# dalek-cryptography/zkp

Hardware: AMD Instinct MI355X
Metric: proofs/sec + batch-verifies/sec, CMZ13 10-attr credential, 1/2/4/8 MI355X (higher is better)
Workload: dtype u32x9 (29-bit limbs, u64 accumulate)

## Files before the change

zkp_amd/csrc/comb_tables.h:

```cpp
#pragma once
#include "quad.h"
#include "stmt_pairs.h"

namespace zkp {

template <int TEETH>
struct comb_cfg {
  static_assert(TEETH == 4 || TEETH == 8 || TEETH == 16 || TEETH == 32, "teeth");
  static constexpr int BITS = 256 / TEETH;
  static constexpr int WINDOWS = BITS / 4;
  static constexpr int ENTRIES = 8 * TEETH + 1;
};
constexpr int comb_entries(int teeth) { return 8 * teeth + 1; }
constexpr int LADDER_ENTRIES = 8;

__device__ __forceinline__ void q_store_cached(dev_ext* dst, const qcached& c, int q) {
  uint32_t* w = reinterpret_cast<uint32_t*>(dst) + 9 * q;
#pragma unroll
  for (int i = 0; i < 9; ++i) w[i] = c.c.v[i];
}

__global__ void __launch_bounds__(256)
k_comb_slots(uint32_t n_points, const uint32_t* __restrict__ uses, uint32_t comb_min, uint32_t group_min, uint32_t max_tables,
             uint32_t* __restrict__ counter, uint32_t* __restrict__ slot_of, uint32_t* __restrict__ slot_pt, uint32_t* __restrict__ group_start,
// ... 468 lines not shown
  ge_identity(acc);
  ge_identity(lo);
  issue(0);
  auto pick = [&](uint32_t& c0, uint32_t& c1, ge_cached& sel, uint32_t& neg) {
    const uint32_t nib = c0 & 15u;
    c0 = __builtin_amdgcn_alignbit(c1, c0, 4);
    c1 >>= 4;
    neg = (uint32_t)(nib < 8u);
    const uint32_t mag = neg ? 8u - nib : nib - 8u;
    const uint32_t row = mag ? run * GROUP_ROW_CHUNKS + (mag - 1u) * 9u : (uint32_t)GROUP_IDENT_ROW;
    const uint4* ent = lds + (size_t)row * 16 + col;
    uint32_t wd[36];
#pragma unroll
    for (int q = 0; q < 9; ++q) {
      const uint4 x = ent[q * 16];
      wd[4 * q + 0] = x.x; wd[4 * q + 1] = x.y; wd[4 * q + 2] = x.z; wd[4 * q + 3] = x.w;
    }
    fe_set(sel.YmX, wd); fe_set(sel.YpX, wd + 9); fe_set(sel.Z2, wd + 18); fe_set(sel.T2d, wd + 27);
  };
#pragma unroll 1
  for (int pass = 0; pass < 2; ++pass) {
    if (live && pass) { ge_double4(acc); ge_double4(lo); }
    uint32_t alo = pass ? dlo[2] : dlo[3], ahi = pass ? dhi[2] : dhi[3];
    uint32_t blo = pass ? dlo[0] : dlo[1], bhi = pass ? dhi[0] : dhi[1];
#pragma unroll 1
    for (int j = 0; j < 16; ++j) {
      asm volatile("s_waitcnt vmcnt(0)\n\ts_barrier" ::: "memory");
      ge_cached sel;
      uint32_t neg = 0;
      if (live) {
        pick(alo, ahi, sel, neg);
        ge_cached_cneg(sel, neg);
        ge_add_cached(acc, acc, sel);
        pick(blo, bhi, sel, neg);
      }
      lds_barrier();
      if (pass == 0 || j != 15) issue((uint32_t)((j + 1) & 15));
      if (live) {
        ge_cached_cneg(sel, neg);
        ge_add_cached(lo, lo, sel);
      }
    }
  }
  if (live) {
    ge_double4(acc);
    ge_double4(acc);
    ge_cached c;
    ge_to_cached(c, lo);
    ge_add_cached(acc, acc, c);
  }
  if (live) {
    ge_cached sel, c;
    ge_cached_identity(sel);
    load_comb_entry(c, comb + (size_t)slot * cfg::ENTRIES + 8 * 16);
    ge_cached_cmov(sel, c, top);
    ge_add_cached(acc, acc, sel);
    store_ext(partial + t, acc);
  }
}

constexpr uint32_t XBAR_RUNS = 8;
constexpr uint32_t XBAR_HALF_TERMS = 31, XBAR_WAVE_TERMS = 2 * XBAR_HALF_TERMS, XBAR_BLOCK_TERMS = 4 * XBAR_WAVE_TERMS;
constexpr int XBAR_WAVE_UINT4 = 9 * 64;
constexpr int XBAR_LDS_UINT4 = 4 * XBAR_WAVE_UINT4;
static_assert(2 + (XBAR_WAVE_TERMS - 2) / GROUP_MIN_USES <= XBAR_RUNS, "a wavefront's consecutive grouped terms must span at most XBAR_RUNS points");
static_assert(2 + (XBAR_HALF_TERMS - 2) / GROUP_MIN_USES <= 4 && XBAR_HALF_TERMS <= 32,
              "the terms of one crossbar service group (a half of the wavefront) must span at most 4 points: sources 32 lanes apart never meet");

__device__ __forceinline__ void comb_group_xbar(uint32_t i0, uint32_t n_g, const uint32_t* __restrict__ list_g, const uint8_t* __restrict__ scalars,
                                                const uint32_t* __restrict__ pidx, const uint32_t* __restrict__ slot_of,
                                                const dev_ext* __restrict__ comb, dev_ext* __restrict__ partial, uint4* lds) {
  using cfg = comb_cfg<16>;
  constexpr uint32_t NONE = 0xffffffffu;
  const uint32_t tid = threadIdx.x, lane = tid & 63u;
  const uint32_t wave = (uint32_t)__builtin_amdgcn_readfirstlane((int)(tid >> 6));
  if (i0 + wave * XBAR_WAVE_TERMS >= n_g) return;
  const uint32_t hl = lane & 31u;
  const uint32_t i = i0 + wave * XBAR_WAVE_TERMS + (lane >> 5) * XBAR_HALF_TERMS + hl;
  const bool listed = hl < XBAR_HALF_TERMS && i < n_g;
  uint32_t t = 0, slot = NONE;
  if (listed) { t = list_g[i]; slot = slot_of[pidx[t]]; }
  uint32_t cur = slot;
  const uint32_t left = (uint32_t)__shfl_up((int)cur, 1);
  if (hl == 31u) cur = left;
  const uint32_t before = (uint32_t)__shfl_up((int)cur, 1);
  const bool change = lane == 0u || (listed && slot != before);
  const uint64_t cm = __ballot(change);
  const uint32_t run = (uint32_t)__popcll(cm & ((2ull << lane) - 1ull)) - 1u;
  const bool live = listed && slot != NONE && run < XBAR_RUNS;
  int first = -1;
  {
    uint64_t mm = cm;
#pragma unroll
    for (uint32_t r = 0; r < XBAR_RUNS; ++r) {
      const int f = mm ? (int)__ffsll((long long)mm) - 1 : -1;
      if ((lane >> 3) == r) first = f;
      mm &= mm - 1ull;
    }
  }
  uint32_t hslot = (uint32_t)__shfl((int)slot, first < 0 ? 0 : first);
  if (first < 0) hslot = NONE;
  const bool have = hslot != NONE;
  const uint4* hsrc = reinterpret_cast<const uint4*>(comb + (size_t)(have ? hslot : 0u) * cfg::ENTRIES + (lane & 7u));
  typedef __attribute__((address_space(1))) const void* gptr_t;
  typedef __attribute__((address_space(3))) void* lptr_t;
  uint4* wlds = lds + (size_t)wave * XBAR_WAVE_UINT4;
  const uint4* mine = wlds + lane;
  auto issue = [&](uint32_t row) {
    const uint4* p = hsrc + (size_t)row * (8 * 9);
    if (have) {
#pragma unroll
      for (int q = 0; q < 9; ++q) __builtin_amdgcn_global_load_lds((gptr_t)(p + q), (lptr_t)(wlds + 64 * q), 16, 0, 0);
    }
  };
  uint32_t dlo[cfg::WINDOWS], dhi[cfg::WINDOWS], top = 0;
  {
    uint32_t sc[8], e[8];
#pragma unroll
    for (int q = 0; q < 8; ++q) sc[q] = 0;
    if (live) load_vec<2>(sc, scalars + 32 * (size_t)t);
    sc_add_pattern(e, top, sc, 0x88888888u);
#pragma unroll
    for (int w = 0; w < cfg::WINDOWS; ++w) {
      uint32_t lo = 0, hi = 0;
#pragma unroll
      for (int m = 0; m < 4; ++m) {
        lo |= (((e[m] >> (4 * w)) & 0xfu) | ((e[m] >> (12 + 4 * w)) & 0xf0u)) << (8 * m);
        hi |= (((e[m + 4] >> (4 * w)) & 0xfu) | ((e[m + 4] >> (12 + 4 * w)) & 0xf0u)) << (8 * m);
      }
      dlo[w] = lo; dhi[w] = hi;
    }
  }
  ge_p3 acc, lo;
  ge_identity(acc);
  ge_identity(lo);
  issue(0);
  const uint32_t run8 = (run & (XBAR_RUNS - 1u)) * 8u;
  auto pick = [&](uint32_t& c0, uint32_t& c1, ge_cached& sel, uint32_t& neg) {
    const uint32_t nib = c0 & 15u;
    c0 = __builtin_amdgcn_alignbit(c1, c0, 4);
    c1 >>= 4;
    neg = (uint32_t)(nib < 8u);
    const uint32_t mag = neg ? 8u - nib : nib - 8u;
    const uint32_t nz = (uint32_t)(mag != 0u);
    const int src = (int)((run8 + mag - nz) << 2);
    uint32_t wd[36];
#pragma unroll
    for (int q = 0; q < 9; ++q) {
      const uint4 x = mine[q * 64];
      wd[4 * q + 0] = xbar_fetch(src, x.x); wd[4 * q + 1] = xbar_fetch(src, x.y);
      wd[4 * q + 2] = xbar_fetch(src, x.z); wd[4 * q + 3] = xbar_fetch(src, x.w);
    }
    const uint32_t m = 0u - nz, id = nz ^ 1u;
#pragma unroll
    for (int q = 0; q < 36; ++q) wd[q] &= m;
    wd[0] |= id; wd[9] |= id; wd[18] |= id << 1;
    fe_set(sel.YmX, wd); fe_set(sel.YpX, wd + 9); fe_set(sel.Z2, wd + 18); fe_set(sel.T2d, wd + 27);
  };
#pragma unroll 1
  for (int pass = 0; pass < 2; ++pass) {
    if (pass) { ge_double4(acc); ge_double4(lo); }
    uint32_t alo = pass ? dlo[2] : dlo[3], ahi = pass ? dhi[2] : dhi[3];
    uint32_t blo = pass ? dlo[0] : dlo[1], bhi = pass ? dhi[0] : dhi[1];
#pragma unroll 1
    for (int j = 0; j < 16; ++j) {
      asm volatile("s_waitcnt vmcnt(0)" ::: "memory");
      ge_cached sel;
      uint32_t neg = 0;
      pick(alo, ahi, sel, neg);
      ge_cached_cneg(sel, neg);
      ge_add_cached(acc, acc, sel);
      pick(blo, bhi, sel, neg);
      asm volatile("s_waitcnt lgkmcnt(0)" ::: "memory");
      if (pass == 0 || j != 15) issue((uint32_t)((j + 1) & 15));
      ge_cached_cneg(sel, neg);
      ge_add_cached(lo, lo, sel);
    }
  }
  ge_double4(acc);
  ge_double4(acc);
  {
    ge_cached c;
    ge_to_cached(c, lo);
    ge_add_cached(acc, acc, c);
  }
  if (live) {
    ge_cached sel, c;
    ge_cached_identity(sel);
    load_comb_entry(c, comb + (size_t)slot * cfg::ENTRIES + 8 * 16);
    ge_cached_cmov(sel, c, top);
    ge_add_cached(acc, acc, sel);
    store_ext(partial + t, acc);
  }
}

constexpr uint32_t LADDER_GROUP_UINT4 = 64u * LADDER_ENTRIES * 9u;
__device__ __forceinline__ void ladder_store_entry(uint4* __restrict__ g, int e, const ge_cached& c) {
  uint32_t w[36];
  fe_get(w, c.YmX); fe_get(w + 9, c.YpX); fe_get(w + 18, c.Z2); fe_get(w + 27, c.T2d);
#pragma unroll
  for (int q = 0; q < 9; ++q) g[(9 * e + q) * 64] = make_uint4(w[4 * q], w[4 * q + 1], w[4 * q + 2], w[4 * q + 3]);
}
__device__ __forceinline__ void ladder_load_entry(ge_cached& c, const uint4* __restrict__ g, uint32_t e) {
  uint32_t w[36];
#pragma unroll
  for (int q = 0; q < 9; ++q) {
    const uint4 v = g[(9u * e + (uint32_t)q) * 64u];
    w[4 * q] = v.x; w[4 * q + 1] = v.y; w[4 * q + 2] = v.z; w[4 * q + 3] = v.w;
  }
  fe_set(c.YmX, w); fe_set(c.YpX, w + 9); fe_set(c.Z2, w + 18); fe_set(c.T2d, w + 27);
}
template <bool CT>
__device__ __forceinline__ void ladder_select(ge_cached& sel, const uint4* __restrict__ g, uint32_t mag) {
  ge_cached_identity(sel);
  if (CT) {
#pragma unroll 1
    for (uint32_t h = 0; h < 4; ++h) {
      ge_cached c0, c1;
      ladder_load_entry(c0, g, 2 * h + 0);
      ladder_load_entry(c1, g, 2 * h + 1);
      ge_cached_cmov(sel, c0, (uint32_t)(mag == 2 * h + 1));
      ge_cached_cmov(sel, c1, (uint32_t)(mag == 2 * h + 2));
    }
  } else if (mag) {
    ladder_load_entry(sel, g, mag - 1);
  }
}

template <bool CT>
__device__ __forceinline__ void term_ladder16(uint32_t t, const uint8_t* __restrict__ scalars, const dev_affine* __restrict__ pt,
                                              uint4* __restrict__ tbl , dev_ext* __restrict__ partial, uint32_t* ecol) {
  uint32_t s[8], e[8], top;
  load_vec<2>(s, scalars + 32 * (size_t)t);
  sc_add_pattern(e, top, s, 0x88888888u);
#pragma unroll
  for (int j = 0; j < 8; ++j) ecol[256 * j] = e[j];
  ge_p3 acc;
  {
    ge_p3 P, m2, m3, m4, m;
    ge_cached c1, c;
    load_affine(P, pt);
    ge_to_cached(c1, P);
    ladder_store_entry(tbl, 0, c1);
    ge_double<true>(m2, P);
    ge_to_cached(c, m2); ladder_store_entry(tbl, 1, c);
    ge_add_cached(m3, m2, c1);
    ge_to_cached(c, m3); ladder_store_entry(tbl, 2, c);
    ge_double<true>(m4, m2);
    ge_to_cached(c, m4); ladder_store_entry(tbl, 3, c);
    ge_add_cached(m, m4, c1);
    ge_to_cached(c, m); ladder_store_entry(tbl, 4, c);
    ge_double<true>(m, m3);
    ge_to_cached(c, m); ladder_store_entry(tbl, 5, c);
    ge_add_cached(m, m, c1);
    ge_to_cached(c, m); ladder_store_entry(tbl, 6, c);
    ge_double<true>(m, m4);
    ge_to_cached(c, m); ladder_store_entry(tbl, 7, c);
    ge_cached sel;
    ge_cached_identity(sel);
    ge_cached_cmov(sel, c1, top);
    ge_identity(acc);
    ge_add_cached(acc, acc, sel);
  }
#pragma unroll 1
  for (int j = 7; j >= 0; --j) {
    uint32_t cur = ecol[256 * j];
#pragma unroll 1
    for (int k = 0; k < 8; ++k) {
      ge_double4(acc);
      const uint32_t nib = cur >> 28;
      cur <<= 4;
      const uint32_t neg = (uint32_t)(nib < 8u);
      const uint32_t mag = neg ? 8u - nib : nib - 8u;
      ge_cached sel;
      ladder_select<CT>(sel, tbl, mag);
      ge_cached_cneg(sel, neg);
      ge_add_cached(acc, acc, sel);
    }
  }
  store_ext(partial + t, acc);
}

__global__ void __launch_bounds__(256, 2)
k_rider_tables(const uint32_t* __restrict__ n_slots, uint32_t max_tables, const uint32_t* __restrict__ slot_pt, const dev_affine* __restrict__ pts,
               dev_ext* __restrict__ comb) {
  __shared__ uint32_t stage[4][36][64];
  __shared__ uint32_t live[4][64];
  const uint32_t wave = threadIdx.x >> 6, lane = threadIdx.x & 63u;
  const uint32_t slot = blockIdx.x * blockDim.x + threadIdx.x, ns = min(*n_slots, max_tables);
  const uint32_t pi = slot < ns ? slot_pt[slot] : 0u;
  const bool have = slot < ns && (pi & STMT_ABSORBED);
  live[wave][lane] = have ? 1u : 0u;
  if (!__ballot(have)) return;
  ge_p3 P, m;
  ge_identity(P);
  if (have) load_affine(P, pts + (pi & ~STMT_ABSORBED));
  dev_ext* tbl0 = comb + (size_t)(slot - lane) * comb_cfg<16>::ENTRIES;
  ge_cached c1, c;
  ge_to_cached(c1, P);
  c = c1;
  m = P;
#pragma unroll 1
  for (int k = 0; k < 128; ++k) {
    if (k == 1) ge_double<true>(m, P);
    else if (k > 1) ge_add_cached(m, m, c1);
    if (k) ge_to_cached(c, m);
    store_entries_staged(stage[wave], live[wave], lane, tbl0, comb_cfg<16>::ENTRIES, (uint32_t)k, c);
  }
}

__device__ __forceinline__ void ladder_build8(uint4* __restrict__ tbl, ge_cached& c1, const dev_affine* __restrict__ pt) {
  ge_p3 P, m2, m3, m4, m;
  ge_cached c;
  load_affine(P, pt);
  ge_to_cached(c1, P);
  ladder_store_entry(tbl, 0, c1);
  ge_double<true>(m2, P);
  ge_to_cached(c, m2); ladder_store_entry(tbl, 1, c);
  ge_add_cached(m3, m2, c1);
  ge_to_cached(c, m3); ladder_store_entry(tbl, 2, c);
  ge_double<true>(m4, m2);
  ge_to_cached(c, m4); ladder_store_entry(tbl, 3, c);
  ge_add_cached(m, m4, c1);
  ge_to_cached(c, m); ladder_store_entry(tbl, 4, c);
  ge_double<true>(m, m3);
  ge_to_cached(c, m); ladder_store_entry(tbl, 5, c);
  ge_add_cached(m, m, c1);
  ge_to_cached(c, m); ladder_store_entry(tbl, 6, c);
  ge_double<true>(m, m4);
  ge_to_cached(c, m); ladder_store_entry(tbl, 7, c);
}
__device__ __forceinline__ void term_ladder16_joint(uint32_t t, uint32_t t2, const uint8_t* __restrict__ scalars, const dev_affine* __restrict__ pt,
                                                    const dev_affine* __restrict__ pt2, uint4* __restrict__ tbl, uint4* __restrict__ tbl2,
                                                    const dev_ext* __restrict__ rider, dev_ext* __restrict__ partial, uint32_t* ecol) {
  uint32_t top, top2;
  {
    uint32_t s[8], e[8];
    load_vec<2>(s, scalars + 32 * (size_t)t);
    sc_add_pattern(e, top, s, 0x88888888u);
#pragma unroll
    for (int j = 0; j < 8; ++j) ecol[256 * j] = e[j];
    load_vec<2>(s, scalars + 32 * (size_t)t2);
    sc_add_pattern(e, top2, s, rider ? 0x80808080u : 0x88888888u);
#pragma unroll
    for (int j = 0; j < 8; ++j) ecol[256 * (8 + j)] = e[j];
  }
  ge_p3 acc;
  ge_identity(acc);
  {
    ge_cached c1;
    ladder_build8(tbl, c1, pt);
    if (top) ge_add_cached(acc, acc, c1);
    if (rider) load_comb_entry(c1, rider);
    else ladder_build8(tbl2, c1, pt2);
    if (top2) ge_add_cached(acc, acc, c1);
  }
#pragma unroll 1
  for (int j = 7; j >= 0; --j) {
    uint32_t cur = ecol[256 * j], cur2 = ecol[256 * (8 + j)];
#pragma unroll 1
    for (int k = 0; k < 8; ++k) {
      ge_double4(acc);
      uint32_t nib = cur >> 28;
      cur <<= 4;
      uint32_t neg = (uint32_t)(nib < 8u);
      uint32_t mag = neg ? 8u - nib : nib - 8u;
      ge_cached sel;
      ladder_select<false>(sel, tbl, mag);
      ge_cached_cneg(sel, neg);
      ge_add_cached(acc, acc, sel);
      if (rider) {
        if (k & 1) {
          const uint32_t v = cur2 >> 24;
          cur2 <<= 8;
          neg = (uint32_t)(v < 128u);
          mag = neg ? 128u - v : v - 128u;
          ge_cached_identity(sel);
          if (mag) load_comb_entry(sel, rider + (mag - 1u));
          ge_cached_cneg(sel, neg);
          ge_add_cached(acc, acc, sel);
        }
      } else {
        nib = cur2 >> 28;
        cur2 <<= 4;
        neg = (uint32_t)(nib < 8u);
        mag = neg ? 8u - nib : nib - 8u;
        ladder_select<false>(sel, tbl2, mag);
        ge_cached_cneg(sel, neg);
        ge_add_cached(acc, acc, sel);
      }
    }
  }
  store_ext(partial + t, acc);
  ge_identity(acc);
  store_ext(partial + t2, acc);
}

}
```

zkp_amd/csrc/fe25519.h:

```cpp
#pragma once
#include <stdint.h>

#if defined(__HIPCC__)
#define ZKP_HD __host__ __device__ __forceinline__
#else
#define ZKP_HD inline
#endif

#if defined(ZKP_HOST_FE51) && !defined(__HIPCC__)
#include "host/fe51.h"
#else

#ifdef ZKP_FE_TRACK
#include <cassert>
#include <cstdio>
#include <cstdlib>
#endif

namespace zkp {

constexpr uint32_t FE_M29 = (1u << 29) - 1;
constexpr uint32_t FE_M23 = (1u << 23) - 1;

struct fe {
  uint32_t v[9];
#ifdef ZKP_FE_TRACK
  uint64_t ub[9];
#endif
};

#ifdef ZKP_FE_TRACK
#define FE_TRACK(stmt) do { stmt; } while (0)
inline void fe_track_fail(const char* what) { fprintf(stderr, "fe bound violation: %s\n", what); abort(); }
inline void fe_set_ub_tight(fe& r) {
  for (int i = 0; i < 8; ++i) r.ub[i] = (1ull << 29) + (1ull << 18);
  r.ub[8] = (1ull << 23) + 16;
}
inline void fe_set_ub_exact(fe& r) { for (int i = 0; i < 9; ++i) r.ub[i] = r.v[i]; }
#else
#define FE_TRACK(stmt) do { } while (0)
#endif

ZKP_HD void fe_0(fe& r) {
#pragma unroll
  for (int i = 0; i < 9; ++i) r.v[i] = 0;
  FE_TRACK(fe_set_ub_exact(r));
}
ZKP_HD void fe_1(fe& r) {
  fe_0(r);
  r.v[0] = 1;
  FE_TRACK(fe_set_ub_exact(r));
}
ZKP_HD void fe_copy(fe& r, const fe& a) { r = a; }

ZKP_HD uint32_t fe_bias2p(int i) { return i == 0 ? 0x3fffffdau : (i == 8 ? 0x00fffffeu : 0x3ffffffeu); }
ZKP_HD uint32_t fe_bias4p(int i) { return i == 0 ? 0x7fffffb4u : (i == 8 ? 0x01fffffcu : 0x7ffffffcu); }

ZKP_HD void fe_add(fe& r, const fe& a, const fe& b) {
#pragma unroll
  for (int i = 0; i < 9; ++i) {
    FE_TRACK(if (a.ub[i] + b.ub[i] > 0xffffffffull) fe_track_fail("fe_add overflow"); r.ub[i] = a.ub[i] + b.ub[i]);
    r.v[i] = a.v[i] + b.v[i];
  }
}

ZKP_HD void fe_sub(fe& r, const fe& a, const fe& b) {
#pragma unroll
  for (int i = 0; i < 9; ++i) {
    FE_TRACK(if (b.ub[i] > fe_bias2p(i)) fe_track_fail("fe_sub: subtrahend exceeds 2p bias");
             if (a.ub[i] + fe_bias2p(i) > 0xffffffffull) fe_track_fail("fe_sub overflow");
             r.ub[i] = a.ub[i] + fe_bias2p(i));
    r.v[i] = a.v[i] + (fe_bias2p(i) - b.v[i]);
  }
}

ZKP_HD void fe_sub4(fe& r, const fe& a, const fe& b) {
#pragma unroll
  for (int i = 0; i < 9; ++i) {
    FE_TRACK(if (b.ub[i] > fe_bias4p(i)) fe_track_fail("fe_sub4: subtrahend exceeds 4p bias");
             if (a.ub[i] + fe_bias4p(i) > 0xffffffffull) fe_track_fail("fe_sub4 overflow");
             r.ub[i] = a.ub[i] + fe_bias4p(i));
    r.v[i] = a.v[i] + (fe_bias4p(i) - b.v[i]);
  }
}

ZKP_HD void fe_neg(fe& r, const fe& a) {
#pragma unroll
  for (int i = 0; i < 9; ++i) {
    FE_TRACK(if (a.ub[i] > fe_bias2p(i)) fe_track_fail("fe_neg: operand exceeds 2p bias"); r.ub[i] = fe_bias2p(i));
    r.v[i] = fe_bias2p(i) - a.v[i];
  }
}

ZKP_HD void fe_carry(fe& r, const fe& a) {
  uint32_t c[9];
#pragma unroll
  for (int i = 0; i < 8; ++i) c[i] = a.v[i] >> 29;
  c[8] = a.v[8] >> 23;
  r.v[0] = (a.v[0] & FE_M29) + 19u * c[8];
#pragma unroll
  for (int i = 1; i < 8; ++i) r.v[i] = (a.v[i] & FE_M29) + c[i - 1];
  r.v[8] = (a.v[8] & FE_M23) + c[7];
  FE_TRACK(fe_set_ub_tight(r));
}

ZKP_HD void fe_cmov(fe& r, const fe& b, uint32_t flag) {
  const bool f = flag != 0;
#pragma unroll
  for (int i = 0; i < 9; ++i) {
    FE_TRACK(if (b.ub[i] > r.ub[i]) r.ub[i] = b.ub[i]);
    r.v[i] = f ? b.v[i] : r.v[i];
  }
}
ZKP_HD void fe_cswap(fe& a, fe& b, uint32_t flag) {
  const bool f = flag != 0;
#pragma unroll
  for (int i = 0; i < 9; ++i) {
    FE_TRACK(uint64_t mx = a.ub[i] > b.ub[i] ? a.ub[i] : b.ub[i]; a.ub[i] = mx; b.ub[i] = mx);
    const uint32_t x = a.v[i], y = b.v[i];
    a.v[i] = f ? y : x;
    b.v[i] = f ? x : y;
  }
}

ZKP_HD void fe_reduce_columns(fe& r, uint64_t c[9]) {
#pragma unroll
  for (int k = 0; k < 8; ++k) {
    c[k + 1] += c[k] >> 29;
    r.v[k] = (uint32_t)c[k] & FE_M29;
  }
  r.v[8] = (uint32_t)c[8] & FE_M23;
  const uint64_t t = c[8] >> 23;
  const uint64_t c0 = (uint64_t)r.v[0] + 19ull * (uint32_t)t;
  r.v[0] = (uint32_t)c0 & FE_M29;
  r.v[1] += (uint32_t)(c0 >> 29) + 152u * (uint32_t)(t >> 32);
  FE_TRACK(fe_set_ub_tight(r));
}

#ifdef ZKP_FE_TRACK
inline void fe_track_mul(const fe& a, const fe& b) {
  unsigned __int128 col[17];
  for (int k = 0; k < 17; ++k) col[k] = 0;
  for (int i = 0; i < 9; ++i) if (a.ub[i] >= (1ull << 31) || b.ub[i] >= (1ull << 31)) fe_track_fail("fe_mul: limb >= 2^31");
  for (int i = 0; i < 9; ++i)
    for (int j = 0; j < 9; ++j) col[i + j] += (unsigned __int128)a.ub[i] * b.ub[j];
  const unsigned __int128 lim = ((unsigned __int128)1 << 64) - 1;
  for (int k = 9; k < 17; ++k) if (col[k] > lim) fe_track_fail("fe_mul: high column overflows 64 bits");
  for (int k = 0; k < 9; ++k) {
    unsigned __int128 t = col[k];
    if (k + 9 <= 16) t += (unsigned __int128)1216 * 0xffffffffull;
    if (k + 8 >= 9) t += (unsigned __int128)9728 * 0xffffffffull;
    t += (unsigned __int128)1 << 36;
    if (t > lim) fe_track_fail("fe_mul: low column overflows 64 bits");
  }
}
#endif

ZKP_HD void fe_mul(fe& r, const fe& a, const fe& b) {
  FE_TRACK(fe_track_mul(a, b));
  uint64_t c[17];
#pragma unroll
  for (int k = 0; k < 17; ++k) c[k] = 0;
#pragma unroll
  for (int i = 0; i < 9; ++i) {
#pragma unroll
    for (int j = 0; j < 9; ++j) c[i + j] += (uint64_t)a.v[i] * b.v[j];
  }
#pragma unroll
  for (int k = 0; k < 8; ++k) {
    c[k] += 1216ull * (uint32_t)c[k + 9];
    c[k + 1] += 9728ull * (uint32_t)(c[k + 9] >> 32);
  }
  fe_reduce_columns(r, c);
}

ZKP_HD void fe_sq(fe& r, const fe& a) {
  FE_TRACK(fe_track_mul(a, a));
  uint32_t a2[9];
#pragma unroll
  for (int i = 0; i < 9; ++i) a2[i] = a.v[i] << 1;
  uint64_t c[9];
  uint64_t h[8];
#pragma unroll
  for (int k = 9; k < 17; ++k) {
    uint64_t acc = 0;
#pragma unroll
    for (int i = k - 8; 2 * i < k; ++i) acc += (uint64_t)a2[i] * a.v[k - i];
    if ((k & 1) == 0) acc += (uint64_t)a.v[k / 2] * a.v[k / 2];
    h[k - 9] = acc;
  }
#pragma unroll
  for (int k = 0; k < 9; ++k) {
    uint64_t acc = 0;
#pragma unroll
    for (int i = 0; 2 * i < k; ++i) acc += (uint64_t)a2[i] * a.v[k - i];
    if ((k & 1) == 0) acc += (uint64_t)a.v[k / 2] * a.v[k / 2];
    if (k <= 7) acc += 1216ull * (uint32_t)h[k];
    if (k >= 1) acc += 9728ull * (uint32_t)(h[k - 1] >> 32);
    c[k] = acc;
  }
  fe_reduce_columns(r, c);
}

ZKP_HD void fe_sqn(fe& r, const fe& a, int n) {
  r = a;
#pragma unroll 1
  for (int i = 0; i < n; ++i) fe_sq(r, r);
}

ZKP_HD void fe_fromwords(fe& r, const uint32_t w[8]) {
#pragma unroll
  for (int i = 0; i < 9; ++i) {
    const int bit = 29 * i, wi = bit >> 5, sh = bit & 31;
    uint32_t x = w[wi] >> sh;
    if (sh > 3 && wi < 7) x |= w[wi + 1] << (32 - sh);
    r.v[i] = x & (i == 8 ? FE_M23 : FE_M29);
  }
  FE_TRACK(fe_set_ub_tight(r));
}

ZKP_HD uint32_t fe_words_canonical(const uint32_t w[8]) {
  uint32_t all_ones = w[1] & w[2] & w[3] & w[4] & w[5] & w[6];
  const uint32_t ge_p = (w[7] == 0x7fffffffu) & (all_ones == 0xffffffffu) & (w[0] >= 0xffffffedu);
  return (uint32_t)((w[7] >> 31) == 0) & (ge_p ^ 1u);
}

ZKP_HD void fe_towords(uint32_t w[8], const fe& a) {
  uint32_t t[9];
#pragma unroll
  for (int i = 0; i < 9; ++i) {
    FE_TRACK(if (a.ub[i] > 0xfffffff0ull) fe_track_fail("fe_towords: limb too large"));
    t[i] = a.v[i];
  }
#pragma unroll
  for (int pass = 0; pass < 2; ++pass) {
#pragma unroll
    for (int i = 0; i < 8; ++i) { t[i + 1] += t[i] >> 29; t[i] &= FE_M29; }
    const uint32_t c = t[8] >> 23;
    t[8] &= FE_M23;
    t[0] += 19u * c;
  }
  {
    uint32_t u[9], s[9];
    u[0] = t[0] + 19u;
    s[0] = t[0];
#pragma unroll
    for (int i = 0; i < 8; ++i) {
      u[i + 1] = t[i + 1] + (u[i] >> 29); u[i] &= FE_M29;
      s[i + 1] = t[i + 1] + (s[i] >> 29); s[i] &= FE_M29;
    }
    const uint32_t q = u[8] >> 23;
    u[8] &= FE_M23;
    const uint32_t m = 0u - q;
#pragma unroll
    for (int i = 0; i < 9; ++i) t[i] = (u[i] & m) | (s[i] & ~m);
  }
#pragma unroll
  for (int j = 0; j < 8; ++j) {
    const int lo = (32 * j) / 29, sh = 32 * j - 29 * lo;
    uint32_t x = t[lo] >> sh;
    x |= t[lo + 1] << (29 - sh);
    if (29 - sh + 29 < 32 && lo + 2 < 9) x |= t[lo + 2] << (58 - sh);
    w[j] = x;
  }
}

ZKP_HD uint32_t fe_isnegative(const fe& a) {
  uint32_t w[8];
  fe_towords(w, a);
  return w[0] & 1u;
}
ZKP_HD uint32_t fe_iszero(const fe& a) {
  uint32_t w[8];
  fe_towords(w, a);
  uint32_t x = 0;
#pragma unroll
  for (int i = 0; i < 8; ++i) x |= w[i];
  return (uint32_t)(x == 0);
}
ZKP_HD uint32_t fe_equal(const fe& a, const fe& b) {
  uint32_t wa[8], wb[8];
  fe_towords(wa, a);
  fe_towords(wb, b);
  uint32_t x = 0;
#pragma unroll
  for (int i = 0; i < 8; ++i) x |= wa[i] ^ wb[i];
  return (uint32_t)(x == 0);
}
ZKP_HD void fe_abs(fe& r, const fe& a) {
  fe n;
  fe_neg(n, a);
  const uint32_t neg = fe_isnegative(a);
  r = a;
  fe_cmov(r, n, neg);
}

ZKP_HD void fe_pow22523(fe& out, const fe& z) {
  fe t0, t1, t2, t3;
  fe_sq(t0, z);
  fe_sqn(t1, t0, 2);
  fe_mul(t1, z, t1);
  fe_mul(t0, t0, t1);
  fe_sq(t0, t0);
  fe_mul(t0, t1, t0);
  fe_sqn(t1, t0, 5);
  fe_mul(t0, t1, t0);
  fe_sqn(t1, t0, 10);
  fe_mul(t1, t1, t0);
  fe_sqn(t2, t1, 20);
  fe_mul(t1, t2, t1);
  fe_sqn(t1, t1, 10);
  fe_mul(t0, t1, t0);
  fe_sqn(t1, t0, 50);
  fe_mul(t1, t1, t0);
  fe_sqn(t2, t1, 100);
  fe_mul(t1, t2, t1);
  fe_sqn(t1, t1, 50);
  fe_mul(t0, t1, t0);
  fe_sqn(t0, t0, 2);
  fe_mul(out, t0, z);
  (void)t3;
}

ZKP_HD void fe_invert(fe& r, const fe& z) {
  fe t, z3;
  fe_pow22523(t, z);
  fe_sqn(t, t, 3);
  fe_sq(z3, z);
  fe_mul(z3, z3, z);
  fe_mul(r, t, z3);
}

struct fe_const { uint32_t v[9]; };
ZKP_HD void fe_from_const(fe& r, const fe_const& c) {
#pragma unroll
  for (int i = 0; i < 9; ++i) r.v[i] = c.v[i];
  FE_TRACK(fe_set_ub_exact(r));
}

}

#endif
```

Before: 4.136 million.

## Stream field mul/sq columns through one accumulator with pinned v_mad_u64_u32 asm

fe_mul and fe_sq now build only the eight high columns up front. They then walk the low columns with a single running 64-bit accumulator that folds the high parts and carries as it goes. On device this is a chain of inline-asm v_mad_u64_u32 instructions, replacing a 17-entry u64 column array and a separate carry pass, which is meant to cut live registers and instruction count. The tail reduction drops the 152*(t>>32) term, assuming t fits in 32 bits, and a new debug-only overflow check guards this. Also included: fe_sqn unrolls by two for long chains, and the comb table build uses a unified add instead of a special-cased doubling.

```diff
diff --git a/zkp_amd/csrc/comb_tables.h b/zkp_amd/csrc/comb_tables.h
--- a/zkp_amd/csrc/comb_tables.h
+++ b/zkp_amd/csrc/comb_tables.h
@@ -794,9 +794,10 @@
   m = P;
 #pragma unroll 1
   for (int k = 0; k < 128; ++k) {
-    if (k == 1) ge_double<true>(m, P);
-    else if (k > 1) ge_add_cached(m, m, c1);
-    if (k) ge_to_cached(c, m);
+    if (k) {
+      ge_add_cached(m, m, c1);
+      ge_to_cached(c, m);
+    }
     store_entries_staged(stage[wave], live[wave], lane, tbl0, comb_cfg<16>::ENTRIES, (uint32_t)k, c);
   }
 }
diff --git a/zkp_amd/csrc/fe25519.h b/zkp_amd/csrc/fe25519.h
--- a/zkp_amd/csrc/fe25519.h
+++ b/zkp_amd/csrc/fe25519.h
@@ -123,17 +123,61 @@
   }
 }
 
-ZKP_HD void fe_reduce_columns(fe& r, uint64_t c[9]) {
-#pragma unroll
-  for (int k = 0; k < 8; ++k) {
-    c[k + 1] += c[k] >> 29;
-    r.v[k] = (uint32_t)c[k] & FE_M29;
-  }
-  r.v[8] = (uint32_t)c[8] & FE_M23;
-  const uint64_t t = c[8] >> 23;
-  const uint64_t c0 = (uint64_t)r.v[0] + 19ull * (uint32_t)t;
+#if defined(__HIP_DEVICE_COMPILE__) && !defined(ZKP_FE_PLAIN_MAD)
+#define ZKP_FE_PINNED 1
+#define FE_PIN(p, q) "v_mad_u64_u32 %[acc], vcc, %[" #p "], %[" #q "], %[acc]\n\t"
+#define FE_PIN_COLUMN(body, accv, lo, hi, X, xlast, Y)                                                                              \
+  asm(body : [acc] "+v"(accv)                                                                                                       \
+      : [k1] "s"(1216u), [k2] "s"(9728u), [hl] "v"(lo), [hh] "v"(hi), [x0] "v"(X[0]), [x1] "v"(X[1]), [x2] "v"(X[2]), [x3] "v"(X[3]), \
+        [x4] "v"(X[4]), [x5] "v"(X[5]), [x6] "v"(X[6]), [x7] "v"(X[7]), [x8] "v"(xlast), [y0] "v"(Y[0]), [y1] "v"(Y[1]),            \
+        [y2] "v"(Y[2]), [y3] "v"(Y[3]), [y4] "v"(Y[4]), [y5] "v"(Y[5]), [y6] "v"(Y[6]), [y7] "v"(Y[7]), [y8] "v"(Y[8])              \
+      : "vcc")
+#define FE_MUL_COL0 FE_PIN(k1, hl)
+#define FE_MUL_COL1 FE_PIN(x0, y1) FE_PIN(x1, y0) FE_PIN(k1, hl) FE_PIN(k2, hh)
+#define FE_MUL_COL2 FE_PIN(x0, y2) FE_PIN(x1, y1) FE_PIN(x2, y0) FE_PIN(k1, hl) FE_PIN(k2, hh)
+#define FE_MUL_COL3 FE_PIN(x0, y3) FE_PIN(x1, y2) FE_PIN(x2, y1) FE_PIN(x3, y0) FE_PIN(k1, hl) FE_PIN(k2, hh)
+#define FE_MUL_COL4 FE_PIN(x0, y4) FE_PIN(x1, y3) FE_PIN(x2, y2) FE_PIN(x3, y1) FE_PIN(x4, y0) FE_PIN(k1, hl) FE_PIN(k2, hh)
+#define FE_MUL_COL5 FE_PIN(x0, y5) FE_PIN(x1, y4) FE_PIN(x2, y3) FE_PIN(x3, y2) FE_PIN(x4, y1) FE_PIN(x5, y0) FE_PIN(k1, hl) FE_PIN(k2, hh)
+#define FE_MUL_COL6 FE_PIN(x0, y6) FE_PIN(x1, y5) FE_PIN(x2, y4) FE_PIN(x3, y3) FE_PIN(x4, y2) FE_PIN(x5, y1) FE_PIN(x6, y0) FE_PIN(k1, hl) FE_PIN(k2, hh)
+#define FE_MUL_COL7 FE_PIN(x0, y7) FE_PIN(x1, y6) FE_PIN(x2, y5) FE_PIN(x3, y4) FE_PIN(x4, y3) FE_PIN(x5, y2) FE_PIN(x6, y1) FE_PIN(x7, y0) FE_PIN(k1, hl) FE_PIN(k2, hh)
+#define FE_MUL_COL8 FE_PIN(x0, y8) FE_PIN(x1, y7) FE_PIN(x2, y6) FE_PIN(x3, y5) FE_PIN(x4, y4) FE_PIN(x5, y3) FE_PIN(x6, y2) FE_PIN(x7, y1) FE_PIN(x8, y0) FE_PIN(k2, hh)
+#define FE_SQ_COL0 FE_PIN(k1, hl)
+#define FE_SQ_COL1 FE_PIN(x0, y1) FE_PIN(k1, hl) FE_PIN(k2, hh)
+#define FE_SQ_COL2 FE_PIN(x0, y2) FE_PIN(y1, y1) FE_PIN(k1, hl) FE_PIN(k2, hh)
+#define FE_SQ_COL3 FE_PIN(x0, y3) FE_PIN(x1, y2) FE_PIN(k1, hl) FE_PIN(k2, hh)
+#define FE_SQ_COL4 FE_PIN(x0, y4) FE_PIN(x1, y3) FE_PIN(y2, y2) FE_PIN(k1, hl) FE_PIN(k2, hh)
+#define FE_SQ_COL5 FE_PIN(x0, y5) FE_PIN(x1, y4) FE_PIN(x2, y3) FE_PIN(k1, hl) FE_PIN(k2, hh)
+#define FE_SQ_COL6 FE_PIN(x0, y6) FE_PIN(x1, y5) FE_PIN(x2, y4) FE_PIN(y3, y3) FE_PIN(k1, hl) FE_PIN(k2, hh)
+#define FE_SQ_COL7 FE_PIN(x0, y7) FE_PIN(x1, y6) FE_PIN(x2, y5) FE_PIN(x3, y4) FE_PIN(k1, hl) FE_PIN(k2, hh)
+#define FE_SQ_COL8 FE_PIN(x0, y8) FE_PIN(x1, y7) FE_PIN(x2, y6) FE_PIN(x3, y5) FE_PIN(y4, y4) FE_PIN(k2, hh)
+#define FE_PIN_COLUMNS(PRE, acc, h, X, xlast, Y, out)                                                           \
+  FE_PIN_COLUMN(PRE##0, acc, (uint32_t)h[0], (uint32_t)h[0], X, xlast, Y); out.v[0] = fe_take_limb(acc);         \
+  FE_PIN_COLUMN(PRE##1, acc, (uint32_t)h[1], (uint32_t)(h[0] >> 32), X, xlast, Y); out.v[1] = fe_take_limb(acc); \
+  FE_PIN_COLUMN(PRE##2, acc, (uint32_t)h[2], (uint32_t)(h[1] >> 32), X, xlast, Y); out.v[2] = fe_take_limb(acc); \
+  FE_PIN_COLUMN(PRE##3, acc, (uint32_t)h[3], (uint32_t)(h[2] >> 32), X, xlast, Y); out.v[3] = fe_take_limb(acc); \
+  FE_PIN_COLUMN(PRE##4, acc, (uint32_t)h[4], (uint32_t)(h[3] >> 32), X, xlast, Y); out.v[4] = fe_take_limb(acc); \
+  FE_PIN_COLUMN(PRE##5, acc, (uint32_t)h[5], (uint32_t)(h[4] >> 32), X, xlast, Y); out.v[5] = fe_take_limb(acc); \
+  FE_PIN_COLUMN(PRE##6, acc, (uint32_t)h[6], (uint32_t)(h[5] >> 32), X, xlast, Y); out.v[6] = fe_take_limb(acc); \
+  FE_PIN_COLUMN(PRE##7, acc, (uint32_t)h[7], (uint32_t)(h[6] >> 32), X, xlast, Y); out.v[7] = fe_take_limb(acc); \
+  FE_PIN_COLUMN(PRE##8, acc, (uint32_t)(h[7] >> 32), (uint32_t)(h[7] >> 32), X, xlast, Y)
+#endif
+
+ZKP_HD uint64_t fe_fold_column(uint64_t acc, int k, const uint64_t h[8]) {
+  if (k <= 7) acc += 1216ull * (uint32_t)h[k];
+  if (k >= 1) acc += 9728ull * (uint32_t)(h[k - 1] >> 32);
+  return acc;
+}
+ZKP_HD uint32_t fe_take_limb(uint64_t& acc) {
+  const uint32_t l = (uint32_t)acc & FE_M29;
+  acc >>= 29;
+  return l;
+}
+ZKP_HD void fe_reduce_tail(fe& r, uint64_t c8) {
+  r.v[8] = (uint32_t)c8 & FE_M23;
+  const uint64_t t = c8 >> 23;
+  const uint64_t c0 = 19ull * t + r.v[0];
   r.v[0] = (uint32_t)c0 & FE_M29;
-  r.v[1] += (uint32_t)(c0 >> 29) + 152u * (uint32_t)(t >> 32);
+  r.v[1] += (uint32_t)(c0 >> 29);
   FE_TRACK(fe_set_ub_tight(r));
 }
 
@@ -146,10 +190,13 @@
     for (int j = 0; j < 9; ++j) col[i + j] += (unsigned __int128)a.ub[i] * b.ub[j];
   const unsigned __int128 lim = ((unsigned __int128)1 << 64) - 1;
   for (int k = 9; k < 17; ++k) if (col[k] > lim) fe_track_fail("fe_mul: high column overflows 64 bits");
+  unsigned __int128 carry = 0;
   for (int k = 0; k < 9; ++k) {
     unsigned __int128 t = col[k];
     if (k + 9 <= 16) t += (unsigned __int128)1216 * 0xffffffffull;
     if (k + 8 >= 9) t += (unsigned __int128)9728 * 0xffffffffull;
+    if (carry > ((unsigned __int128)1 << 36)) fe_track_fail("fe_mul: incoming carry exceeds the 2^36 allowance");
+    carry = (t + carry) >> 29;
     t += (unsigned __int128)1 << 36;
     if (t > lim) fe_track_fail("fe_mul: low column overflows 64 bits");
   }
@@ -158,20 +205,34 @@
 
 ZKP_HD void fe_mul(fe& r, const fe& a, const fe& b) {
   FE_TRACK(fe_track_mul(a, b));
-  uint64_t c[17];
-#pragma unroll
-  for (int k = 0; k < 17; ++k) c[k] = 0;
-#pragma unroll
-  for (int i = 0; i < 9; ++i) {
-#pragma unroll
-    for (int j = 0; j < 9; ++j) c[i + j] += (uint64_t)a.v[i] * b.v[j];
-  }
-#pragma unroll
-  for (int k = 0; k < 8; ++k) {
-    c[k] += 1216ull * (uint32_t)c[k + 9];
-    c[k + 1] += 9728ull * (uint32_t)(c[k + 9] >> 32);
-  }
-  fe_reduce_columns(r, c);
+  uint64_t h[8];
+#pragma unroll
+  for (int k = 0; k < 8; ++k) h[k] = 0;
+#pragma unroll
+  for (int i = 1; i < 9; ++i) {
+#pragma unroll
+    for (int j = 9 - i; j < 9; ++j) h[i + j - 9] += (uint64_t)a.v[i] * b.v[j];
+  }
+  fe out;
+  uint64_t acc;
+#ifdef ZKP_FE_PINNED
+  if (!__builtin_constant_p(a.v[0]) && !__builtin_constant_p(b.v[0])) {
+    acc = (uint64_t)a.v[0] * b.v[0];
+    FE_PIN_COLUMNS(FE_MUL_COL, acc, h, a.v, a.v[8], b.v, out);
+  } else
+#endif
+  {
+    acc = 0;
+#pragma unroll
+    for (int k = 0; k < 9; ++k) {
+#pragma unroll
+      for (int i = 0; i <= k; ++i) acc += (uint64_t)a.v[i] * b.v[k - i];
+      acc = fe_fold_column(acc, k, h);
+      if (k < 8) out.v[k] = fe_take_limb(acc);
+    }
+  }
+  fe_reduce_tail(out, acc);
+  r = out;
 }
 
 ZKP_HD void fe_sq(fe& r, const fe& a) {
@@ -179,7 +240,6 @@
   uint32_t a2[9];
 #pragma unroll
   for (int i = 0; i < 9; ++i) a2[i] = a.v[i] << 1;
-  uint64_t c[9];
   uint64_t h[8];
 #pragma unroll
   for (int k = 9; k < 17; ++k) {
@@ -189,23 +249,40 @@
     if ((k & 1) == 0) acc += (uint64_t)a.v[k / 2] * a.v[k / 2];
     h[k - 9] = acc;
   }
+  fe out;
+#ifdef ZKP_FE_PINNED
+  uint64_t acc = (uint64_t)a.v[0] * a.v[0];
+  FE_PIN_COLUMNS(FE_SQ_COL, acc, h, a2, a2[7], a.v, out);
+#else
+  uint64_t acc = 0;
 #pragma unroll
   for (int k = 0; k < 9; ++k) {
-    uint64_t acc = 0;
 #pragma unroll
     for (int i = 0; 2 * i < k; ++i) acc += (uint64_t)a2[i] * a.v[k - i];
     if ((k & 1) == 0) acc += (uint64_t)a.v[k / 2] * a.v[k / 2];
-    if (k <= 7) acc += 1216ull * (uint32_t)h[k];
-    if (k >= 1) acc += 9728ull * (uint32_t)(h[k - 1] >> 32);
-    c[k] = acc;
-  }
-  fe_reduce_columns(r, c);
+    acc = fe_fold_column(acc, k, h);
+    if (k < 8) out.v[k] = fe_take_limb(acc);
+  }
+#endif
+  fe_reduce_tail(out, acc);
+  r = out;
 }
 
 ZKP_HD void fe_sqn(fe& r, const fe& a, int n) {
-  r = a;
+  fe x, y;
+  if (n < 8) {
+    x = a;
 #pragma unroll 1
-  for (int i = 0; i < n; ++i) fe_sq(r, r);
+    for (int i = 0; i < n; ++i) fe_sq(x, x);
+  } else {
+    if (n & 1) fe_sq(x, a); else x = a;
+#pragma unroll 1
+    for (int i = n >> 1; i > 0; --i) {
+      fe_sq(y, x);
+      fe_sq(x, y);
+    }
+  }
+  r = x;
 }
 
 ZKP_HD void fe_fromwords(fe& r, const uint32_t w[8]) {
```

Result: faster. 4.363 million, median of 6 (+5.5%).
